# maybeLx/MVSFormerPlusPlus

Hardware: AMD Instinct MI355X
Metric: ref-views/sec at 1152x1536 N=5 D=192 4-stage; achieved HBM GB/s vs peak (higher is better)
Workload: dtype fp16 operands/storage, fp32 accumulate (every stage; 1-2 fp16 MFMA terms)

## Files before the change

mvsformerplusplus_amd/csrc/conv_bf16x3_kernels.hip:

```cpp
#include <map>
#include <mutex>
#include <type_traits>
#include <utility>

#include "conv_cfg.h"
#include "split_format.h"

#ifndef MVS_ABL
#define MVS_ABL 0
#endif
#ifndef MVS_WPF
#define MVS_WPF 1
#endif
#ifndef MVS_MSPLIT
#define MVS_MSPLIT 1
#endif
#ifndef MVS_MSPLIT_MIN_MREP
#define MVS_MSPLIT_MIN_MREP 4
#endif
#ifndef MVS_PERSIST
#define MVS_PERSIST 1
#endif
#ifndef MVS_PERSIST_PFD
#define MVS_PERSIST_PFD 1
// ... 613 lines not shown
}

#ifndef MVS_CONV_LOADER
#define MVS_CONV_LOADER 0
#endif
#if MVS_CONV_LOADER
__device__ float4 g_conv_zero_line[4];

template <class Cfg>
struct BfConvLd {
    static constexpr int OPT = BfConv<Cfg>::OPT;
    static constexpr int IMG = ((int)BfConv<Cfg>::LDS_BYTES + 255) / 256 * 256;
    static constexpr int NPC = (Cfg::NVOX + 63) / 64;
    static constexpr int NP = OPT * NPC;
    static constexpr size_t LDS_BYTES = (size_t)2 * IMG;
    static constexpr bool ENABLED = MVS_CONV_LOADER && BfConv<Cfg>::F16 && !BfConv<Cfg>::PERSIST && Cfg::KD == 3;
};

template <class Cfg>
__global__ __launch_bounds__(320) void conv3d_mfma_f16_loader_kernel(const _Float16* __restrict__ x, const void* wp, const float* __restrict__ bias,
                                                                     _Float16* __restrict__ y, int D, int H, int W, int OD, int OH, int OW,
                                                                     int relu, int tiles_x, int tiles_y, int ntiles) {
    constexpr int CIN = Cfg::CIN, COUT = Cfg::COUT, SD = Cfg::SD, SH = Cfg::SH, SW = Cfg::SW, TD = Cfg::TD, TH = Cfg::TH, CH = Cfg::CH;
    constexpr int IH = Cfg::IH, IW = Cfg::IW, MREP = Cfg::MREP, NREP = Cfg::NREP, NPASS = Cfg::NPASS, NVOX = Cfg::NVOX;
    constexpr int NSTEP = BfConv<Cfg>::NSTEP, SB = BfConv<Cfg>::SB, PLANE = BfConv<Cfg>::PLANE;
    constexpr int IMG = BfConvLd<Cfg>::IMG, NPC = BfConvLd<Cfg>::NPC, NP = BfConvLd<Cfg>::NP;
    static_assert(BfConv<Cfg>::F16 && SB == 16, "fp16 activations: 16 bytes per voxel and octet");
    HIP_DYNAMIC_SHARED(float4, lds4)
    char* lds = reinterpret_cast<char*>(lds4);
    const int tid = (int)threadIdx.x, lane = tid & 63;
    const int wave = __builtin_amdgcn_readfirstlane(tid >> 6);
    const int b = (int)blockIdx.y;
    const int nblk = (int)gridDim.x, per = (ntiles + nblk - 1) / nblk;
    const int t_begin = (int)xcd_remap(blockIdx.x, (unsigned)nblk) * per;
    const int t_end = t_begin + per < ntiles ? t_begin + per : ntiles;
    if (t_begin >= t_end) return;
    const int nchunk = (t_end - t_begin) * NPASS;
    const char* xb = reinterpret_cast<const char*>(x) + (size_t)b * D * H * W * CIN * 2;

    if (wave == 4) {
        const char* zero = reinterpret_cast<const char*>(g_conv_zero_line);
        int crd[NPC];
        int rel[NPC];
#pragma unroll
        for (int k = 0; k < NPC; ++k) {
            const int v = 64 * k + lane;
            const int dx = v % IW, t2 = v / IW, dy = t2 % IH, dz = t2 / IH;
            crd[k] = v < NVOX ? (dz << 16 | dy << 8 | dx) : -1;
            rel[k] = ((dz * H + dy) * W + dx) * (CIN * 2);
        }
        auto issue = [&](int c, int buf) {
            const int tile = t_begin + c / NPASS, pass = c - (c / NPASS) * NPASS;
            const int tx = tile % tiles_x, t1 = tile / tiles_x;
            const int ty = t1 % tiles_y, tz = t1 / tiles_y;
            const int iz0 = tz * TD * SD - Cfg::PD, iy0 = ty * TH * SH - 1, ix0 = tx * 16 * SW - 1;
            const long long base = ((long long)(iz0 * H + iy0) * W + ix0) * (CIN * 2) + pass * (CH * 2);
            char* img = lds + buf * IMG;
#pragma unroll
            for (int k = 0; k < NPC; ++k) {
                if (crd[k] < 0) continue;
                const int z = iz0 + (crd[k] >> 16), yy = iy0 + ((crd[k] >> 8) & 0xff), xx = ix0 + (crd[k] & 0xff);
                const bool ok = MVS_ABL != 1 && (unsigned)z < (unsigned)D && (unsigned)yy < (unsigned)H && (unsigned)xx < (unsigned)W;
#pragma unroll
                for (int oc = 0; oc < BfConvLd<Cfg>::OPT; ++oc) {
                    const char* src = ok ? xb + base + rel[k] + oc * 16 : zero;
                    MVS_GLOBAL_LOAD_LDS16(src, img + oc * PLANE + k * 1024);
                }
            }
        };
        issue(0, 0);
        MVS_WAIT_VMEM();
        __syncthreads();
        for (int c = 0; c < nchunk; ++c) {
            if (c + 1 < nchunk) issue(c + 1, (c + 1) & 1);
            MVS_WAIT_VMEM();
            __syncthreads();
        }
        return;
    }

    float sat_amax = 0.0f;
    const int li = lane & 15, g = lane >> 4;
    constexpr int MSPLIT = CfgSplit<Cfg>::MSPLIT, MREP_ALL = CfgSplit<Cfg>::MREP_ALL;
    const int mb0 = (wave % MSPLIT) * MREP, rowgrp = wave / MSPLIT;
    int voxbase[NREP];
#pragma unroll
    for (int nb = 0; nb < NREP; ++nb) {
        const int nbg = rowgrp * NREP + nb;
        const int oz = nbg / TH, oy = nbg % TH;
        voxbase[nb] = (((oz * SD) * IH + oy * SH) * IW + li * SW) * SB;
    }
    float4 bb[MREP];
#pragma unroll
    for (int mb = 0; mb < MREP; ++mb) {
        const int co = 16 * (mb0 + mb) + 4 * g;
        bb[mb] = co < COUT ? *reinterpret_cast<const float4*>(bias + co) : make_float4(0.0f, 0.0f, 0.0f, 0.0f);
    }
    _Float16* yb = y + (size_t)b * OD * OH * OW * COUT;
    f32x4 acc[MREP][NREP];
    __syncthreads();
    for (int c = 0; c < nchunk; ++c) {
        const int tile = t_begin + c / NPASS, pass = c - (c / NPASS) * NPASS;
        const char* cur = lds + (c & 1) * IMG;
        const bf16x8* wq = reinterpret_cast<const bf16x8*>(wp) + ((size_t)pass * NSTEP * MREP_ALL + mb0) * 2 * 64 + lane;
        bf16x8 ah[MVS_WPF + 1][MREP], al[MVS_WPF + 1][MREP];
        bf_conv_preload_w<Cfg>(wq, ah, al);
        if (pass == 0) {
#pragma unroll
            for (int mb = 0; mb < MREP; ++mb)
#pragma unroll
                for (int nb = 0; nb < NREP; ++nb) acc[mb][nb] = (f32x4){0.0f, 0.0f, 0.0f, 0.0f};
        }
        bf_conv_contract<Cfg>(wq, cur, voxbase, g, acc, ah, al);
        if (pass == NPASS - 1) {
            const int tx = tile % tiles_x, t1 = tile / tiles_x;
            const int ty = t1 % tiles_y, tz = t1 / tiles_y;
            const int oz0 = tz * TD, oy0 = ty * TH, ox0 = tx * 16;
#pragma unroll
            for (int nb = 0; nb < NREP; ++nb) {
                const int nbg = rowgrp * NREP + nb;
                const int oz = oz0 + nbg / TH, oy = oy0 + nbg % TH, ox = ox0 + li;
                if (!(oz < OD && oy < OH && ox < OW)) continue;
                _Float16* o = yb + (((size_t)oz * OH + oy) * OW + ox) * COUT;
#pragma unroll
                for (int mb = 0; mb < MREP; ++mb) {
                    const int co = 16 * (mb0 + mb) + 4 * g;
                    if (co >= COUT) continue;
                    float4 v = make_float4(acc[mb][nb][0] + bb[mb].x, acc[mb][nb][1] + bb[mb].y, acc[mb][nb][2] + bb[mb].z, acc[mb][nb][3] + bb[mb].w);
                    if (relu) { v.x = fmaxf(v.x, 0.0f); v.y = fmaxf(v.y, 0.0f); v.z = fmaxf(v.z, 0.0f); v.w = fmaxf(v.w, 0.0f); }
                    *reinterpret_cast<f16x4*>(o + co) = f16_pack4(v, sat_amax);
                }
            }
        }
        __syncthreads();
    }
    sat::commit(sat_amax);
}
#endif

template <class Cfg>
struct BfDeconv {
    static constexpr int OPT = Cfg::CIN / 8;
#ifndef MVS_DECONV_PLANES
#define MVS_DECONV_PLANES 1
#endif
    static constexpr bool F16 = CfgFmt<Cfg>::F16;
    static constexpr int RUNB = F16 ? 16 : 32;
    static constexpr int SB = F16 ? 16 : (MVS_DECONV_PLANES ? 32 : Cfg::S * 4);
    static constexpr int PLANE = F16 ? (Cfg::NVOX * 16 + 255) / 256 * 256 + bf_f16_plane_shift(1)
                                     : (MVS_DECONV_PLANES ? (Cfg::NVOX * 32 + 255) / 256 * 256 + 16 : 32);
    static constexpr size_t LDS_BYTES = (F16 || MVS_DECONV_PLANES) ? (size_t)OPT * PLANE : Cfg::LDS_BYTES;
};

template <class Cfg>
__device__ __forceinline__ void bf_deconv_load_step(int st, int ntap, int pd, int ph, int pw, int g, const bf16x8* wq, const char* ldsb,
                                                    const int* voxbase, bf16x8* ah, bf16x8* al, bf16x8* bh, bf16x8* bl) {
    constexpr int SD = Cfg::SD, OPT = BfDeconv<Cfg>::OPT;
    const int o = 4 * st + g;
    int ti = o / OPT;
    const int oc = o - ti * OPT;
    ti = ti < ntap ? ti : ntap - 1;
    const int nkw = pw ? 2 : 1, nkh = ph ? 2 : 1;
    const int a_w = ti % nkw;
    ti /= nkw;
    const int a_h = ti % nkh, a_d = ti / nkh;
    const int od = (SD == 2) ? (pd ? 1 - a_d : 0) : 1 - a_d;
    const int oh = ph ? 1 - a_h : 0, ow = pw ? 1 - a_w : 0;
    const int ldsoff = ((od * Cfg::LH + oh) * Cfg::LW + ow) * BfDeconv<Cfg>::SB + oc * BfDeconv<Cfg>::PLANE;
#pragma unroll
    for (int mb = 0; mb < Cfg::MREP; ++mb) {
        if (MVS_ABL == 2 && st > 1) continue;
        ah[mb] = wq[(size_t)((st * CfgSplit<Cfg>::MREP_ALL + mb) * 2) * 64];
        al[mb] = wq[(size_t)((st * CfgSplit<Cfg>::MREP_ALL + mb) * 2 + 1) * 64];
    }
#pragma unroll
    for (int nb = 0; nb < Cfg::NREP; ++nb) {
        if (MVS_ABL == 3 && st > 1) continue;
        bh[nb] = *reinterpret_cast<const bf16x8*>(ldsb + voxbase[nb] + ldsoff);
        if constexpr (!BfDeconv<Cfg>::F16) bl[nb] = *reinterpret_cast<const bf16x8*>(ldsb + voxbase[nb] + ldsoff + 16);
    }
}

template <class Cfg, bool SPLIT>
__global__ __launch_bounds__(256) void deconv3d_mfma_bf16x3_kernel(const float* __restrict__ x, const void* wp, const float* __restrict__ bias,
                                                                   const float* __restrict__ skip, float* __restrict__ y,
                                                                   const float* __restrict__ prob_w, const float* __restrict__ prob_b,
                                                                   float* __restrict__ logits, int D, int H, int W, int tiles_x,
                                                                   int tiles_y, int ntiles, int relu) {
    float sat_amax = 0.0f;
    constexpr int CIN = Cfg::CIN, COUT = Cfg::COUT, SD = Cfg::SD, TDM = Cfg::TDM, THM = Cfg::THM;
    constexpr int LH = Cfg::LH, LW = Cfg::LW, MREP = Cfg::MREP, NREP = Cfg::NREP;
    constexpr int OPT = BfDeconv<Cfg>::OPT, SB = BfDeconv<Cfg>::SB;
    const float lo_clamp = relu ? 0.0f : -INFINITY;
    HIP_DYNAMIC_SHARED(float4, lds4)
    char* ldsb = reinterpret_cast<char*>(lds4);
    const int tid = (int)threadIdx.x, lane = tid & 63, wave = tid >> 6;
    const int li = lane & 15, g = lane >> 4;
    start_stagger(2048);
    prio_kernel_begin();
    int tile = (int)xcd_remap(blockIdx.x, (unsigned)ntiles);
    const int b = (int)blockIdx.y;
    const int tx = tile % tiles_x;
    tile /= tiles_x;
    const int ty = tile % tiles_y, tz = tile / tiles_y;
    const int mz0 = tz * TDM, my0 = ty * THM, mx0 = tx * 16;
    const int OD = D * SD, OH = 2 * H, OW = 2 * W;

    constexpr bool F16 = BfDeconv<Cfg>::F16;
    constexpr int EB = F16 ? 2 : 4, RUNB = BfDeconv<Cfg>::RUNB;
    const char* xb = reinterpret_cast<const char*>(x) + (size_t)b * D * H * W * CIN * EB;
    {
        int zrel;
        const __amdgpu_buffer_rsrc_t xrs = bf_make_rsrc_z(xb, mz0 - Cfg::ZO, D, H, W, (unsigned)(CIN * EB), zrel);
        BfTileWalk<LW, LH, OPT, RUNB> wk(tid, zrel, my0, mx0, H, W, CIN * EB, 0u);
        int ldso = (tid / OPT) * SB + (tid % OPT) * BfDeconv<Cfg>::PLANE;
        for (int e = tid; e < Cfg::NVOX * OPT; e += 256) {
            const bool ok = MVS_ABL != 1 && wk.inside(mz0 - Cfg::ZO, my0, mx0, D, H, W);
            const unsigned voff = ok ? wk.off : BF_OOB;
            const float4 u = bf_buf_load16(xrs, voff, 0);
            if constexpr (F16) {
                *reinterpret_cast<float4*>(ldsb + ldso) = u;
            } else {
                const float4 v = bf_buf_load16(xrs, voff, 16);
                stage_to_lds<SPLIT>(ldsb + ldso, u, v);
            }
            wk.advance();
            ldso += (256 / OPT) * SB;
        }
    }
    __syncthreads();

    constexpr int MSPLIT = CfgSplit<Cfg>::MSPLIT, MREP_ALL = CfgSplit<Cfg>::MREP_ALL;
    const int mb0 = (wave % MSPLIT) * MREP, rowgrp = wave / MSPLIT;
    int voxbase[NREP];
#pragma unroll
    for (int nb = 0; nb < NREP; ++nb) {
        const int nbg = rowgrp * NREP + nb;
        const int mz = nbg / THM, my = nbg % THM;
        voxbase[nb] = (((mz + Cfg::ZO) * LH + my) * LW + li) * SB;
    }
    float* yb = reinterpret_cast<float*>(reinterpret_cast<char*>(y) + (size_t)b * OD * OH * OW * COUT * EB);
    const float* sb = skip ? reinterpret_cast<const float*>(reinterpret_cast<const char*>(skip) + (size_t)b * OD * OH * OW * COUT * EB) : nullptr;
    const bf16x8* wq = reinterpret_cast<const bf16x8*>(wp) + (size_t)mb0 * 2 * 64 + lane;

    constexpr bool PAIR = COUT == 8;
    constexpr int NCLS = (SD == 2 ? 2 : 1) * 4;
    constexpr int NIT = PAIR ? NCLS / 2 : NCLS;
    float4 skp[NIT][NREP][MREP];
    if (sb) {
#pragma unroll
        for (int it = 0; it < NIT; ++it) {
            const int cls = PAIR ? 2 * it : it;
            const int pw = PAIR ? 1 : (cls & 1), ph = (cls >> 1) & 1, pd = (SD == 2) ? (cls >> 2) : 0;
#pragma unroll
            for (int nb = 0; nb < NREP; ++nb) {
                const int nbg = rowgrp * NREP + nb;
                const int mz = mz0 + nbg / THM, my = my0 + nbg % THM, mx = mx0 + li;
                const bool inside = mz < D && my < H && mx < W;
                const int oz = mz * SD + pd, oy = 2 * my + ph, ox = PAIR ? 2 * mx + (g >> 1) : 2 * mx + pw;
#pragma unroll
                for (int mb = 0; mb < MREP; ++mb) {
                    const int co = PAIR ? 4 * (g & 1) : 16 * (mb0 + mb) + 4 * g;
                    const size_t sidx = (((size_t)oz * OH + oy) * OW + ox) * COUT;
                    const float* sv = sb + sidx;
                    if constexpr (F16) {
                        const float2 raw = !(inside && co < COUT) ? make_float2(0.0f, 0.0f)
                                                                  : *reinterpret_cast<const float2*>(reinterpret_cast<const _Float16*>(sb) + sidx + co);
                        skp[it][nb][mb] = make_float4(raw.x, raw.y, 0.0f, 0.0f);
                        continue;
                    }
                    skp[it][nb][mb] = !(inside && co < COUT) ? make_float4(0.0f, 0.0f, 0.0f, 0.0f)
                                      : SPLIT ? split_raw_quad(sv + (co & ~7), (co >> 2) & 1) : *reinterpret_cast<const float4*>(sv + co);
                }
            }
        }
    }
#pragma unroll
    for (int cls = 0; cls < NCLS; cls += PAIR ? 2 : 1) {
        const int it = PAIR ? cls / 2 : cls;
        const int pw = PAIR ? 1 : (cls & 1), ph = (cls >> 1) & 1, pd = (SD == 2) ? (cls >> 2) : 0;
        f32x4 acc[MREP][NREP];
#pragma unroll
        for (int mb = 0; mb < MREP; ++mb)
#pragma unroll
            for (int nb = 0; nb < NREP; ++nb) acc[mb][nb] = (f32x4){0.0f, 0.0f, 0.0f, 0.0f};
        const int ntap = ((SD == 2) ? (pd ? 2 : 1) : 3) * (ph ? 2 : 1) * (pw ? 2 : 1);
        const int nst = MVS_ABL == 6 ? 1 : (ntap * OPT + 3) / 4;
        bf16x8 ah0[MREP], al0[MREP], bh0[NREP], bl0[NREP], ah1[MREP], al1[MREP], bh1[NREP], bl1[NREP];
        prio_contract_begin();
        bf_deconv_load_step<Cfg>(0, ntap, pd, ph, pw, g, wq, ldsb, voxbase, ah0, al0, bh0, bl0);
#pragma unroll 1
        for (int st = 0; st + 1 < nst; st += 2) {
            bf_deconv_load_step<Cfg>(st + 1, ntap, pd, ph, pw, g, wq, ldsb, voxbase, ah1, al1, bh1, bl1);
            __builtin_amdgcn_sched_barrier(0);
            bf_mfma_step<MREP, NREP, F16>(ah0, al0, bh0, bl0, acc);
            bf_deconv_load_step<Cfg>(st + 2 < nst ? st + 2 : nst - 1, ntap, pd, ph, pw, g, wq, ldsb, voxbase, ah0, al0, bh0, bl0);
            __builtin_amdgcn_sched_barrier(0);
            bf_mfma_step<MREP, NREP, F16>(ah1, al1, bh1, bl1, acc);
        }
        if (nst & 1) bf_mfma_step<MREP, NREP, F16>(ah0, al0, bh0, bl0, acc);
        prio_contract_end();
        wq += (size_t)nst * MREP_ALL * 2 * 64;

#pragma unroll
        for (int nb = 0; nb < NREP; ++nb) {
            const int nbg = rowgrp * NREP + nb;
            const int mz = mz0 + nbg / THM, my = my0 + nbg % THM, mx = mx0 + li;
            const bool inside = mz < D && my < H && mx < W;
            if (!inside && !(PAIR && prob_w != nullptr) && !SPLIT) continue;
            if (PAIR) {
                const int oz = mz * SD + pd, oy = 2 * my + ph, ox = 2 * mx + (g >> 1), co = 4 * (g & 1);
                const size_t off = (((size_t)oz * OH + oy) * OW + ox) * COUT + co;
                const float4 bb = *reinterpret_cast<const float4*>(bias + co);
                float4 v = make_float4(fmaxf(acc[0][nb][0] + bb.x, lo_clamp), fmaxf(acc[0][nb][1] + bb.y, lo_clamp), fmaxf(acc[0][nb][2] + bb.z, lo_clamp),
                                       fmaxf(acc[0][nb][3] + bb.w, lo_clamp));
                if (sb && inside) {
                    const float4 sk = F16 ? f16_quad_to_f32(skp[it][nb][0]) : SPLIT ? split_join_quad(skp[it][nb][0]) : skp[it][nb][0];
                    v.x += sk.x; v.y += sk.y; v.z += sk.z; v.w += sk.w;
                }
                if (prob_w != nullptr) {
                    const float4 pw4 = *reinterpret_cast<const float4*>(prob_w + co);
                    float part = v.x * pw4.x;
                    part += v.y * pw4.y;
                    part += v.z * pw4.z;
                    part += v.w * pw4.w;
                    part += __shfl_xor(part, 16);
                    if ((g & 1) == 0 && inside && !(MVS_ABL == 5 && part != 12345.678f)) logits[(size_t)b * OD * OH * OW + ((size_t)oz * OH + oy) * OW + ox] = part + prob_b[0];
                } else if (F16) {
                    if (inside) *reinterpret_cast<f16x4*>(reinterpret_cast<_Float16*>(yb) + off) = f16_pack4(v, sat_amax);
                } else if (SPLIT) {
                    split_store_quad(yb + off - co, g, v, inside);
                } else {
                    if (!(MVS_ABL == 5 && v.x != 12345.678f)) *reinterpret_cast<float4*>(yb + off) = v;
                }
                continue;
            }
            const int oz = mz * SD + pd, oy = 2 * my + ph, ox = 2 * mx + pw;
            const size_t off = (((size_t)oz * OH + oy) * OW + ox) * COUT;
#pragma unroll
            for (int mb = 0; mb < MREP; ++mb) {
                const int co = 16 * (mb0 + mb) + 4 * g;
                if (!SPLIT && co >= COUT) continue;
                const float4 bb = *reinterpret_cast<const float4*>(bias + (co < COUT ? co : 0));
                float4 v = make_float4(fmaxf(acc[mb][nb][0] + bb.x, lo_clamp), fmaxf(acc[mb][nb][1] + bb.y, lo_clamp),
                                       fmaxf(acc[mb][nb][2] + bb.z, lo_clamp), fmaxf(acc[mb][nb][3] + bb.w, lo_clamp));
                if (sb) {
                    const float4 sk = F16 ? f16_quad_to_f32(skp[it][nb][mb]) : SPLIT ? split_join_quad(skp[it][nb][mb]) : skp[it][nb][mb];
                    v.x += sk.x; v.y += sk.y; v.z += sk.z; v.w += sk.w;
                }
                if (MVS_ABL == 5 && v.x != 12345.678f) continue;
                if constexpr (F16) *reinterpret_cast<f16x4*>(reinterpret_cast<_Float16*>(yb) + off + co) = f16_pack4(v, sat_amax);
                else if (SPLIT) split_store_quad(yb + off + (co & ~7), g, v, inside && co < COUT);
                else *reinterpret_cast<float4*>(yb + off + co) = v;
            }
        }
    }
    if constexpr (F16) sat::commit(sat_amax);
}

template <class Cfg>
struct BfDeconvP {
    static constexpr bool F16 = CfgFmt<Cfg>::F16;
    static constexpr int OPT = 2, SB = F16 ? 16 : 32, RUNB = SB;
    static constexpr int PLANE = F16 ? (Cfg::NVOX * 16 + 255) / 256 * 256 + bf_f16_plane_shift(1) : (Cfg::NVOX * 32 + 255) / 256 * 256 + 16;
    static constexpr int XBYTES = (2 * PLANE + 255) / 256 * 256;
    static constexpr int NIT = (Cfg::SD == 2 ? 2 : 1) * 2;
    static constexpr int ntap(int it) { return ((Cfg::SD == 2) ? ((it >> 1) ? 2 : 1) : 3) * ((it & 1) ? 2 : 1) * 2; }
    static constexpr int nst(int it) { return (ntap(it) * OPT + 3) / 4; }
    static constexpr int wbase(int it) { return it == 0 ? 0 : wbase(it - 1) + nst(it - 1); }
    static constexpr int WSTEPS = wbase(NIT);
    static constexpr int WBYTES = WSTEPS * 2048;
    static constexpr size_t LDS_BYTES = (size_t)XBYTES + WBYTES;
    static_assert(Cfg::CIN == 16 && Cfg::COUT == 8, "persistent deconv: the 16 -> 8 layer");
    static constexpr int tap_offset(int it, int o) {
        const int pd = (Cfg::SD == 2) ? (it >> 1) : 0, ph = it & 1;
        int ti = o / OPT;
        const int oc = o - ti * OPT;
        ti = ti < ntap(it) ? ti : ntap(it) - 1;
        const int a_w = ti % 2;
        ti /= 2;
        const int nkh = ph ? 2 : 1;
        const int a_h = ti % nkh, a_d = ti / nkh;
        const int od = (Cfg::SD == 2) ? (pd ? 1 - a_d : 0) : 1 - a_d;
        const int oh = ph ? 1 - a_h : 0, ow = 1 - a_w;
        return ((od * Cfg::LH + oh) * Cfg::LW + ow) * SB + oc * PLANE;
    }
};

template <class Cfg, int IT, int T>
__device__ __forceinline__ void bfd_load_step(int g, int lane, const char* ldsx, const char* ldsw, int voxbase0, bf16x8& ah, bf16x8& al, bf16x8* bh,
                                              bf16x8* bl) {
    using P = BfDeconvP<Cfg>;
    static_assert(Cfg::THM % Cfg::NREP == 0, "a wave's rows must stay inside one input plane");
    constexpr int ROWB = Cfg::LW * P::SB;
    constexpr int c0 = P::tap_offset(IT, 4 * T), c1 = P::tap_offset(IT, 4 * T + 1), c2 = P::tap_offset(IT, 4 * T + 2), c3 = P::tap_offset(IT, 4 * T + 3);
    int sel = c0;
    sel = g == 1 ? c1 : sel;
    sel = g == 2 ? c2 : sel;
    sel = g == 3 ? c3 : sel;
    const char* p = ldsx + voxbase0 + sel;
    const char* w = ldsw + (P::wbase(IT) + T) * 2048 + lane * 16;
    ah = *reinterpret_cast<const bf16x8*>(w);
    al = *reinterpret_cast<const bf16x8*>(w + 1024);
#pragma unroll
    for (int nb = 0; nb < Cfg::NREP; ++nb) {
        bh[nb] = *reinterpret_cast<const bf16x8*>(p + nb * ROWB);
        if constexpr (!P::F16) bl[nb] = *reinterpret_cast<const bf16x8*>(p + nb * ROWB + 16);
    }
}

template <class Cfg, int IT, int T>
struct BfDeconvSteps {
    static __device__ __forceinline__ void run(int g, int lane, const char* ldsx, const char* ldsw, int voxbase0, f32x4 (*acc)[Cfg::NREP], bf16x8* a0,
                                               bf16x8* bh0, bf16x8* bl0, bf16x8* a1, bf16x8* bh1, bf16x8* bl1) {
        constexpr int NST = BfDeconvP<Cfg>::nst(IT);
        if constexpr (T < NST) {
            if constexpr (T + 1 < NST) {
                if constexpr ((T & 1) == 0) bfd_load_step<Cfg, IT, T + 1>(g, lane, ldsx, ldsw, voxbase0, a1[0], a1[1], bh1, bl1);
                else bfd_load_step<Cfg, IT, T + 1>(g, lane, ldsx, ldsw, voxbase0, a0[0], a0[1], bh0, bl0);
            }
            __builtin_amdgcn_sched_barrier(0);
            if constexpr ((T & 1) == 0) bf_mfma_step<1, Cfg::NREP, CfgFmt<Cfg>::F16, CfgFmt<Cfg>::ONE>(&a0[0], &a0[1], bh0, bl0, acc);
            else bf_mfma_step<1, Cfg::NREP, CfgFmt<Cfg>::F16, CfgFmt<Cfg>::ONE>(&a1[0], &a1[1], bh1, bl1, acc);
            BfDeconvSteps<Cfg, IT, T + 1>::run(g, lane, ldsx, ldsw, voxbase0, acc, a0, bh0, bl0, a1, bh1, bl1);
        }
    }
};

template <class Cfg, bool SPLIT>
__global__ __launch_bounds__(256) void deconv3d_mfma_bf16x3_persist_kernel(const float* __restrict__ x, const void* wp, const float* __restrict__ bias,
                                                                           const float* __restrict__ skip, float* __restrict__ y,
                                                                           const float* __restrict__ prob_w, const float* __restrict__ prob_b,
                                                                           float* __restrict__ logits, int D, int H, int W, int tiles_x, int tiles_y,
                                                                           int ntiles, int relu) {
    float sat_amax = 0.0f;
    using P = BfDeconvP<Cfg>;
    const float lo_clamp = relu ? 0.0f : -INFINITY;
    constexpr int CIN = Cfg::CIN, COUT = Cfg::COUT, SD = Cfg::SD, TDM = Cfg::TDM, THM = Cfg::THM;
    constexpr int LH = Cfg::LH, LW = Cfg::LW, NREP = Cfg::NREP, NIT = P::NIT, OPT = P::OPT, SB = P::SB;
    HIP_DYNAMIC_SHARED(float4, lds4)
    char* ldsx = reinterpret_cast<char*>(lds4);
    char* ldsw = ldsx + P::XBYTES;
    const int tid = (int)threadIdx.x, lane = tid & 63, wave = tid >> 6;
    const int li = lane & 15, g = lane >> 4;
    const int b = (int)blockIdx.y;
    const int nblk = (int)gridDim.x, per = (ntiles + nblk - 1) / nblk;
    const int t_begin = (int)xcd_remap(blockIdx.x, (unsigned)nblk) * per;
    const int t_end = t_begin + per < ntiles ? t_begin + per : ntiles;
    if (t_begin >= t_end) return;
    const int OD = D * SD, OH = 2 * H, OW = 2 * W;

    for (int e = tid; e < P::WBYTES / 16; e += 256) reinterpret_cast<float4*>(ldsw)[e] = reinterpret_cast<const float4*>(wp)[e];

    constexpr bool F16 = P::F16;
    constexpr int EB = F16 ? 2 : 4;
// ... 65 lines not shown
#pragma unroll
        for (int it = 0; it < NITX; ++it) {
            const int e = tid + it * 256;
            if (e >= NITEM) break;
            const int vox = e / OPT, oc = e - vox * OPT;
            if constexpr (F16) *reinterpret_cast<float4*>(ldsx + vox * SB + oc * P::PLANE) = su[it];
            else stage_to_lds<SPLIT>(ldsx + vox * SB + oc * P::PLANE, su[it], sv[it]);
        }
        __syncthreads();
        if (tile + 1 < t_end) issue_x(tile + 1);

        const int tx = tile % tiles_x;
        const int t1 = tile / tiles_x;
        const int ty = t1 % tiles_y, tz = t1 / tiles_y;
        const int mz0 = tz * TDM, my0 = ty * THM, mx0 = tx * 16;
        float4 outv[NIT][NREP];
        auto run_class = [&](auto itc) {
            constexpr int IT = decltype(itc)::value;
            f32x4 acc[1][NREP];
#pragma unroll
            for (int nb = 0; nb < NREP; ++nb) acc[0][nb] = (f32x4){0.0f, 0.0f, 0.0f, 0.0f};
            bf16x8 a0[2], a1[2], bh0[NREP], bl0[NREP], bh1[NREP], bl1[NREP];
            bfd_load_step<Cfg, IT, 0>(g, lane, ldsx, ldsw, voxbase[0], a0[0], a0[1], bh0, bl0);
            BfDeconvSteps<Cfg, IT, 0>::run(g, lane, ldsx, ldsw, voxbase[0], acc, a0, bh0, bl0, a1, bh1, bl1);
#pragma unroll
            for (int nb = 0; nb < NREP; ++nb)
                outv[IT][nb] = make_float4(fmaxf(acc[0][nb][0] + bb.x, lo_clamp), fmaxf(acc[0][nb][1] + bb.y, lo_clamp), fmaxf(acc[0][nb][2] + bb.z, lo_clamp),
                                           fmaxf(acc[0][nb][3] + bb.w, lo_clamp));
        };
        run_class(std::integral_constant<int, 0>{});
        run_class(std::integral_constant<int, 1>{});
        if constexpr (NIT == 4) {
            run_class(std::integral_constant<int, 2>{});
            run_class(std::integral_constant<int, 3>{});
        }
#pragma unroll
        for (int it = 0; it < NIT; ++it) {
            const int pd = (SD == 2) ? (it >> 1) : 0, ph = it & 1;
#pragma unroll
            for (int nb = 0; nb < NREP; ++nb) {
                const int nbg = wave * NREP + nb;
                const int mz = mz0 + nbg / THM, my = my0 + nbg % THM, mx = mx0 + li;
                const bool inside = mz < D && my < H && mx < W;
                const int oz = mz * SD + pd, oy = 2 * my + ph, ox = 2 * mx + (g >> 1);
                float4 v = outv[it][nb];
                if (sb) {
                    const float4 sk = F16 ? f16_quad_to_f32(skp[it][nb]) : SPLIT ? split_join_quad(skp[it][nb]) : skp[it][nb];
                    v.x += sk.x; v.y += sk.y; v.z += sk.z; v.w += sk.w;
                }
                if (head) {
                    float part = v.x * pw4.x;
                    part += v.y * pw4.y;
                    part += v.z * pw4.z;
                    part += v.w * pw4.w;
                    part += __shfl_xor(part, 16);
                    if ((g & 1) == 0 && inside && !(MVS_ABL == 5 && part != 12345.678f))
                        logits[(size_t)b * OD * OH * OW + ((size_t)oz * OH + oy) * OW + ox] = part + pb;
                } else if (F16) {
                    if (inside) *reinterpret_cast<f16x4*>(reinterpret_cast<_Float16*>(yb) + (((size_t)oz * OH + oy) * OW + ox) * COUT + co) =
                        f16_pack4(v, sat_amax);
                } else if (SPLIT) {
                    split_store_quad(yb + (((size_t)oz * OH + oy) * OW + ox) * COUT, g, v, inside);
                } else if (inside && !(MVS_ABL == 5 && v.x != 12345.678f)) {
                    *reinterpret_cast<float4*>(yb + (((size_t)oz * OH + oy) * OW + ox) * COUT + co) = v;
                }
            }
        }
        if (sb && tile + 1 < t_end) issue_skip(tile + 1);
        __syncthreads();
    }
    if constexpr (F16) sat::commit(sat_amax);
}

static int resident_blocks(const void* func, size_t lds, int threads = 256) {
    static std::mutex mu;
    static std::map<std::pair<const void*, int>, int> cache;
    int dev = 0;
    if (hipGetDevice(&dev) != hipSuccess) return -1;
    std::lock_guard<std::mutex> lock(mu);
    auto it = cache.find(std::make_pair(func, dev));
    if (it != cache.end()) return it->second;
    int per_cu = 0;
    hipDeviceProp_t prop;
    if (lds > 48 * 1024) hipFuncSetAttribute(func, hipFuncAttributeMaxDynamicSharedMemorySize, (int)lds);
    if (hipGetDeviceProperties(&prop, dev) != hipSuccess || hipOccupancyMaxActiveBlocksPerMultiprocessor(&per_cu, func, threads, lds) != hipSuccess || per_cu < 1)
        return -1;
    return cache[std::make_pair(func, dev)] = per_cu * prop.multiProcessorCount;
}

template <class Cfg>
struct BfSplitOf {
    static constexpr bool SPLIT = MVS_MSPLIT && Cfg::MREP >= MVS_MSPLIT_MIN_MREP && Cfg::NREP <= 2 && Cfg::TH % (Cfg::NREP * 2) == 0;
    typedef typename std::conditional<SPLIT, SplitCfg<Cfg, 2>, Cfg>::type type;
};

template <class Cfg, bool SPLIT>
static int launch_conv_bf(const float* x, const void* wp, const float* bias, float* y, int B, int D, int H, int W, int relu, hipStream_t st,
                          float* logits) {
    const int OD = (D + 2 * Cfg::PD - Cfg::KD) / Cfg::SD + 1, OH = (H - 1) / Cfg::SH + 1, OW = (W - 1) / Cfg::SW + 1;
    const int tx = (int)ceil_div(OW, 16), ty = (int)ceil_div(OH, Cfg::TH), tz = (int)ceil_div(OD, Cfg::TD);
    const int ntiles = tx * ty * tz;
    constexpr size_t LDS = BfConv<Cfg>::PERSIST ? BfConv<Cfg>::PERSIST_LDS_BYTES : BfConv<Cfg>::LDS_BYTES;
    if constexpr (BfConv<Cfg>::PERSIST) {
        const int resident = resident_blocks(reinterpret_cast<const void*>(&conv3d_mfma_bf16x3_persist_kernel<Cfg, SPLIT>), LDS);
        if (resident < 1) { set_error("conv3d(bf16x3): occupancy query failed"); return MVS_ERR_LAUNCH; }
        const int nblk = ntiles < resident ? ntiles : resident;
        hipLaunchKernelGGL((conv3d_mfma_bf16x3_persist_kernel<Cfg, SPLIT>), dim3(nblk, B), dim3(256), LDS, st, x, wp, bias, y, logits, D, H, W, OD, OH, OW, relu, tx,
                           ty, ntiles);
        return check_launch("conv3d_mfma_bf16x3_persist_kernel");
    }
    if (logits != nullptr) { set_error("conv3d(bf16x3): the planar single-channel output needs a persistent (Cin = 8) kernel"); return MVS_ERR_UNSUPPORTED; }
#if MVS_CONV_LOADER
    if constexpr (BfConvLd<Cfg>::ENABLED) {
        static const bool off = getenv("MVS_CONV_LOADER_OFF") != nullptr;
        if (!off) {
            constexpr size_t LLDS = BfConvLd<Cfg>::LDS_BYTES;
            const int resident = resident_blocks(reinterpret_cast<const void*>(&conv3d_mfma_f16_loader_kernel<Cfg>), LLDS, 320);
            if (resident < 1) { set_error("conv3d(f16, loader): occupancy query failed"); return MVS_ERR_LAUNCH; }
            const int nblk = ntiles < resident ? ntiles : resident;
            hipLaunchKernelGGL((conv3d_mfma_f16_loader_kernel<Cfg>), dim3(nblk, B), dim3(320), LLDS, st, reinterpret_cast<const _Float16*>(x), wp, bias,
                               reinterpret_cast<_Float16*>(y), D, H, W, OD, OH, OW, relu, tx, ty, ntiles);
            return check_launch("conv3d_mfma_f16_loader_kernel");
        }
    }
#endif
    constexpr size_t TLDS = BfWlds<Cfg>::ENABLED ? BfWlds<Cfg>::LDS_BYTES : LDS;
    if (TLDS > 48 * 1024)
        hipFuncSetAttribute(reinterpret_cast<const void*>(&conv3d_mfma_bf16x3_kernel<Cfg, SPLIT>), hipFuncAttributeMaxDynamicSharedMemorySize, (int)TLDS);
    hipLaunchKernelGGL((conv3d_mfma_bf16x3_kernel<Cfg, SPLIT>), dim3(ntiles, B), dim3(256), TLDS, st, x, wp, bias, y, D, H, W, OD, OH, OW, relu, tx, ty, ntiles);
    return check_launch("conv3d_mfma_bf16x3_kernel");
}

template <class Cfg>
struct BfDeconvSplitOf {
    static constexpr bool SPLIT = MVS_MSPLIT && Cfg::MREP == 2 && Cfg::THM % (Cfg::NREP * 2) == 0;
    typedef typename std::conditional<SPLIT, SplitCfg<Cfg, 2>, Cfg>::type type;
};

template <class Cfg, bool SPLIT>
static int launch_deconv_bf(const float* x, const void* wp, const float* bias, const float* skip, float* y, const float* prob_w,
                            const float* prob_b, float* logits, int B, int D, int H, int W, hipStream_t st, int relu) {
    const int tx = (int)ceil_div(W, 16), ty = (int)ceil_div(H, Cfg::THM), tz = (int)ceil_div(D, Cfg::TDM);
    const int ntiles = tx * ty * tz;
    if constexpr (MVS_PERSIST && Cfg::CIN == 16 && Cfg::COUT == 8) {
        constexpr size_t LDS = BfDeconvP<Cfg>::LDS_BYTES;
        const int resident = resident_blocks(reinterpret_cast<const void*>(&deconv3d_mfma_bf16x3_persist_kernel<Cfg, SPLIT>), LDS);
        if (resident < 1) { set_error("deconv3d(bf16x3): occupancy query failed"); return MVS_ERR_LAUNCH; }
        const int nblk = ntiles < resident ? ntiles : resident;
        hipLaunchKernelGGL((deconv3d_mfma_bf16x3_persist_kernel<Cfg, SPLIT>), dim3(nblk, B), dim3(256), LDS, st, x, wp, bias, skip, y, prob_w, prob_b, logits, D, H,
                           W, tx, ty, ntiles, relu);
        return check_launch("deconv3d_mfma_bf16x3_persist_kernel");
    }
    constexpr size_t DLDS = BfDeconv<Cfg>::LDS_BYTES;
    if (DLDS > 48 * 1024)
        hipFuncSetAttribute(reinterpret_cast<const void*>(&deconv3d_mfma_bf16x3_kernel<Cfg, SPLIT>), hipFuncAttributeMaxDynamicSharedMemorySize, (int)DLDS);
    hipLaunchKernelGGL((deconv3d_mfma_bf16x3_kernel<Cfg, SPLIT>), dim3(ntiles, B), dim3(256), DLDS, st, x, wp, bias, skip, y, prob_w, prob_b,
                       logits, D, H, W, tx, ty, ntiles, relu);
    return check_launch("deconv3d_mfma_bf16x3_kernel");
}

static bool bf_input_fits(const char* who, int Cin, int D, int H, int W, int split) {
    const long long bytes = 12LL * H * W * Cin * (split >= 2 ? 2 : 4);
    if (bytes < (1LL << 31)) return true;
    set_error("%s: twelve z-planes of the input are %lld bytes; the MFMA convolutions address a tile's planes with 32-bit offsets (< 2 GB)", who, bytes);
    return false;
}

int conv3d_dispatch_bf16x3(const float* x, const void* wp, const float* bias, float* y, int B, int Cin, int Cout, int D, int H, int W,
                           int kd, int sd, int sh, int sw, int relu, hipStream_t st, float* logits, int split) {
    if (!bf_input_fits("conv3d(mfma)", Cin, D, H, W, split)) return MVS_ERR_UNSUPPORTED;
#define MVS_X(CI, CO, KD, SD, SH, SW, TD, TH, CH)                                                     \
    if (Cin == CI && Cout == CO && kd == KD && sd == SD && sh == SH && sw == SW) {                    \
        typedef typename BfSplitOf<ConvCfg<CI, CO, KD, SD, SH, SW, TD, TH, CH>>::type K;              \
        if (split == 3) return launch_conv_bf<F16x1Cfg<K>, false>(x, wp, bias, y, B, D, H, W, relu, st, logits); \
        if (split == 2) return launch_conv_bf<F16Cfg<K>, false>(x, wp, bias, y, B, D, H, W, relu, st, logits);   \
        return split ? launch_conv_bf<K, true>(x, wp, bias, y, B, D, H, W, relu, st, logits)          \
                     : launch_conv_bf<K, false>(x, wp, bias, y, B, D, H, W, relu, st, logits);        \
    }
    MVS_CONV_TABLE(MVS_X)
#undef MVS_X
    set_error("conv3d(bf16x3): no kernel for Cin=%d Cout=%d kernel=(%d,3,3) stride=(%d,%d,%d)", Cin, Cout, kd, sd, sh, sw);
    return MVS_ERR_UNSUPPORTED;
}

int deconv3d_dispatch_bf16x3(const float* x, const void* wp, const float* bias, const float* skip, float* y, int B, int Cin, int Cout,
                             int D, int H, int W, int sd, hipStream_t st, const float* prob_w, const float* prob_b, float* logits, int relu, int split) {
    if (prob_w != nullptr && Cout != 8) { set_error("deconv3d(bf16x3): the fused prob head needs Cout == 8"); return MVS_ERR_UNSUPPORTED; }
    if (!bf_input_fits("deconv3d(mfma)", Cin, D, H, W, split)) return MVS_ERR_UNSUPPORTED;
#define MVS_X(CI, CO, SD, TDM, THM)                                                                     \
    if (Cin == CI && Cout == CO && sd == SD) {                                                          \
        typedef typename BfDeconvSplitOf<DeconvCfg<CI, CO, SD, TDM, THM>>::type K;                      \
        if (split == 3) return launch_deconv_bf<F16x1Cfg<K>, false>(x, wp, bias, skip, y, prob_w, prob_b, logits, B, D, H, W, st, relu);    \
        if (split == 2) return launch_deconv_bf<F16Cfg<K>, false>(x, wp, bias, skip, y, prob_w, prob_b, logits, B, D, H, W, st, relu);      \
        return split ? launch_deconv_bf<K, true>(x, wp, bias, skip, y, prob_w, prob_b, logits, B, D, H, W, st, relu)    \
                     : launch_deconv_bf<K, false>(x, wp, bias, skip, y, prob_w, prob_b, logits, B, D, H, W, st, relu);  \
    }
    MVS_DECONV_TABLE(MVS_X)
#undef MVS_X
    set_error("deconv3d(bf16x3): no kernel for Cin=%d Cout=%d stride=(%d,2,2)", Cin, Cout, sd);
    return MVS_ERR_UNSUPPORTED;
}

}

namespace mvs { MVS_DEFINE_SAT_READER(sat_read_conv) }
```

Before: 677.9.

## Fuse deconv parity classes into one compile-time tap walk, drop low weight term

Adds a class-fused path for the stride-(1,2,2) transposed convolutions with 32 or 64 input channels. It walks the 27-tap neighbourhood once, loads each input fragment from LDS a single time, and feeds the MFMAs of all four output parity classes that use that tap, with weights fetched through buffer loads. Separately, when the format uses a single fp16 term, the low weight half is no longer loaded in the per-class path either. The aim is to cut repeated LDS reads and redundant weight loads. In exchange it needs four accumulator sets (more VGPRs, possibly lower occupancy) and a fully unrolled template walk that grows code size.

```diff
diff --git a/mvsformerplusplus_amd/csrc/conv_bf16x3_kernels.hip b/mvsformerplusplus_amd/csrc/conv_bf16x3_kernels.hip
--- a/mvsformerplusplus_amd/csrc/conv_bf16x3_kernels.hip
+++ b/mvsformerplusplus_amd/csrc/conv_bf16x3_kernels.hip
@@ -789,7 +789,7 @@
     static constexpr size_t LDS_BYTES = (F16 || MVS_DECONV_PLANES) ? (size_t)OPT * PLANE : Cfg::LDS_BYTES;
 };
 
-template <class Cfg>
+template <class Cfg, bool ONE = false>
 __device__ __forceinline__ void bf_deconv_load_step(int st, int ntap, int pd, int ph, int pw, int g, const bf16x8* wq, const char* ldsb,
                                                     const int* voxbase, bf16x8* ah, bf16x8* al, bf16x8* bh, bf16x8* bl) {
     constexpr int SD = Cfg::SD, OPT = BfDeconv<Cfg>::OPT;
@@ -808,7 +808,7 @@
     for (int mb = 0; mb < Cfg::MREP; ++mb) {
         if (MVS_ABL == 2 && st > 1) continue;
         ah[mb] = wq[(size_t)((st * CfgSplit<Cfg>::MREP_ALL + mb) * 2) * 64];
-        al[mb] = wq[(size_t)((st * CfgSplit<Cfg>::MREP_ALL + mb) * 2 + 1) * 64];
+        if constexpr (!ONE) al[mb] = wq[(size_t)((st * CfgSplit<Cfg>::MREP_ALL + mb) * 2 + 1) * 64];
     }
 #pragma unroll
     for (int nb = 0; nb < Cfg::NREP; ++nb) {
@@ -818,7 +818,128 @@
     }
 }
 
-template <class Cfg, bool SPLIT>
+#ifndef MVS_DECONV_ONE_TERM
+#define MVS_DECONV_ONE_TERM 1
+#endif
+#ifndef MVS_DECONV_FUSED_DEFAULT
+#define MVS_DECONV_FUSED_DEFAULT 1
+#endif
+#ifndef MVS_DECONV_WPF
+#define MVS_DECONV_WPF 0
+#endif
+template <class Cfg>
+struct BfDeconvF {
+    static constexpr bool ENABLED = Cfg::SD == 1 && (Cfg::CIN == 32 || Cfg::CIN == 64) && Cfg::COUT >= 16;
+    static constexpr bool F16 = CfgFmt<Cfg>::F16, ONE = MVS_DECONV_ONE_TERM && CfgFmt<Cfg>::ONE;
+    static constexpr bool DEFAULT = ENABLED && MVS_DECONV_FUSED_DEFAULT && ONE && Cfg::CIN == 64;
+    static constexpr int SPT = BfDeconv<Cfg>::OPT / 4;
+    static constexpr int NSTEP = 12 * SPT;
+    static constexpr int NW = MVS_DECONV_WPF + 1;
+    static constexpr int ROWB = Cfg::LW * BfDeconv<Cfg>::SB;
+    static constexpr bool uses(int cls, int p) { return ((cls & 2) || (p & 2)) && ((cls & 1) || (p & 1)); }
+    static constexpr int ntap(int cls) { return 3 * ((cls & 2) ? 2 : 1) * ((cls & 1) ? 2 : 1); }
+    static constexpr int wbase(int cls) { return cls == 0 ? 0 : wbase(cls - 1) + ntap(cls - 1) * SPT; }
+    static constexpr int wstep(int cls, int u) {
+        const int p = u / SPT, nkh = (cls & 2) ? 2 : 1, nkw = (cls & 1) ? 2 : 1;
+        const int a_d = p >> 2, a_h = (cls & 2) ? (p >> 1) & 1 : 0, a_w = (cls & 1) ? p & 1 : 0;
+        return wbase(cls) + ((a_d * nkh + a_h) * nkw + a_w) * SPT + u % SPT;
+    }
+    static constexpr int xoff(int u) {
+        const int p = u / SPT, od = 1 - (p >> 2), oh = 1 - ((p >> 1) & 1), ow = 1 - (p & 1);
+        return (((od + 1) * Cfg::LH + oh) * Cfg::LW + ow) * BfDeconv<Cfg>::SB + (u % SPT) * 4 * BfDeconv<Cfg>::PLANE;
+    }
+    static_assert(!ENABLED || Cfg::THM % Cfg::NREP == 0, "a wave's rows must stay inside one input plane");
+};
+
+template <class Cfg, int U, int CLS, int WHICH = 3, int WHEN = 0>
+__device__ __forceinline__ void bfdf_load_w(__amdgpu_buffer_rsrc_t wrs, unsigned wvoff, bf16x8* ah, bf16x8* al) {
+    using P = BfDeconvF<Cfg>;
+    constexpr bool prev = U > 0 && P::uses(CLS, (U > 0 ? U - 1 : 0) / P::SPT);
+    if constexpr (P::uses(CLS, U / P::SPT) && (WHEN == 0 || (WHEN == 1) == prev)) {
+        if (MVS_ABL == 2 && U > 1) return;
+#pragma unroll
+        for (int mb = 0; mb < Cfg::MREP; ++mb) {
+            constexpr int MREP_ALL = CfgSplit<Cfg>::MREP_ALL;
+            const int e = (P::wstep(CLS, U) * MREP_ALL + mb) * 2 * 1024;
+            if constexpr ((WHICH & 2) != 0) ah[mb] = __builtin_bit_cast(bf16x8, __builtin_amdgcn_raw_buffer_load_b128(wrs, (int)wvoff, e, 0));
+            if constexpr ((WHICH & 1) != 0 && !P::ONE) al[mb] = __builtin_bit_cast(bf16x8, __builtin_amdgcn_raw_buffer_load_b128(wrs, (int)wvoff, e + 1024, 0));
+        }
+    }
+}
+template <class Cfg, int U, int WHICH = 3, int WHEN = 0>
+__device__ __forceinline__ void bfdf_load_w_all(__amdgpu_buffer_rsrc_t wrs, unsigned wvoff, bf16x8 (*ah)[Cfg::MREP], bf16x8 (*al)[Cfg::MREP]) {
+    bfdf_load_w<Cfg, U, 0, WHICH, WHEN>(wrs, wvoff, ah[0], al[0]);
+    bfdf_load_w<Cfg, U, 1, WHICH, WHEN>(wrs, wvoff, ah[1], al[1]);
+    bfdf_load_w<Cfg, U, 2, WHICH, WHEN>(wrs, wvoff, ah[2], al[2]);
+    bfdf_load_w<Cfg, U, 3, WHICH, WHEN>(wrs, wvoff, ah[3], al[3]);
+}
+template <class Cfg, int U>
+__device__ __forceinline__ void bfdf_load_x(const char* px, bf16x8* bh, bf16x8* bl) {
+    using P = BfDeconvF<Cfg>;
+#pragma unroll
+    for (int nb = 0; nb < Cfg::NREP; ++nb) {
+        if (MVS_ABL == 3 && U > 1) continue;
+        bh[nb] = *reinterpret_cast<const bf16x8*>(px + P::xoff(U) + nb * P::ROWB);
+        if constexpr (!P::F16) bl[nb] = *reinterpret_cast<const bf16x8*>(px + P::xoff(U) + nb * P::ROWB + 16);
+    }
+}
+template <class Cfg, int U, int TERM, int CLS>
+__device__ __forceinline__ void bfdf_mfma(const bf16x8* ah, const bf16x8* al, const bf16x8* bh, const bf16x8* bl, f32x4 (*acc)[Cfg::NREP]) {
+    using P = BfDeconvF<Cfg>;
+    if constexpr (P::uses(CLS, U / P::SPT)) {
+#pragma unroll
+        for (int mb = 0; mb < Cfg::MREP; ++mb)
+#pragma unroll
+            for (int nb = 0; nb < Cfg::NREP; ++nb) {
+                if constexpr (P::F16)
+                    acc[mb][nb] = __builtin_amdgcn_mfma_f32_16x16x32_f16(__builtin_bit_cast(f16x8, TERM == 0 ? al[mb] : ah[mb]), __builtin_bit_cast(f16x8, bh[nb]),
+                                                                         acc[mb][nb], 0, 0, 0);
+                else
+                    acc[mb][nb] = __builtin_amdgcn_mfma_f32_16x16x32_bf16(TERM == 0 ? al[mb] : ah[mb], TERM == 1 ? bl[nb] : bh[nb], acc[mb][nb], 0, 0, 0);
+            }
+    }
+}
+template <class Cfg, int U, int TERM>
+__device__ __forceinline__ void bfdf_mfma_all(bf16x8 (*ah)[Cfg::MREP], bf16x8 (*al)[Cfg::MREP], const bf16x8* bh, const bf16x8* bl,
+                                              f32x4 (*acc)[Cfg::MREP][Cfg::NREP]) {
+    bfdf_mfma<Cfg, U, TERM, 0>(ah[0], al[0], bh, bl, acc[0]);
+    bfdf_mfma<Cfg, U, TERM, 1>(ah[1], al[1], bh, bl, acc[1]);
+    bfdf_mfma<Cfg, U, TERM, 2>(ah[2], al[2], bh, bl, acc[2]);
+    bfdf_mfma<Cfg, U, TERM, 3>(ah[3], al[3], bh, bl, acc[3]);
+}
+
+template <class Cfg, int U>
+struct BfDeconvFSteps {
+    using P = BfDeconvF<Cfg>;
+    static __device__ __forceinline__ void run(__amdgpu_buffer_rsrc_t wrs, unsigned wvoff, const char* px, f32x4 (*acc)[Cfg::MREP][Cfg::NREP],
+                                               bf16x8 (*ah)[4][Cfg::MREP], bf16x8 (*al)[4][Cfg::MREP], bf16x8 (*bh)[Cfg::NREP], bf16x8 (*bl)[Cfg::NREP]) {
+        constexpr int NSTEP = MVS_ABL == 6 ? 1 : P::NSTEP, WPF = MVS_DECONV_WPF, NW = P::NW;
+        constexpr bool NEXT = U + 1 < NSTEP;
+        if constexpr (U < NSTEP) {
+            if constexpr (WPF > 0 && U + WPF < NSTEP) bfdf_load_w_all<Cfg, U + WPF>(wrs, wvoff, ah[(U + WPF) % NW], al[(U + WPF) % NW]);
+            if constexpr (WPF == 0 && NEXT) bfdf_load_w_all<Cfg, U + 1, 3, 2>(wrs, wvoff, ah[0], al[0]);
+            if constexpr (NEXT) bfdf_load_x<Cfg, U + 1>(px, bh[(U + 1) & 1], bl[(U + 1) & 1]);
+            __builtin_amdgcn_sched_barrier(0);
+            if constexpr (!P::ONE) {
+                bfdf_mfma_all<Cfg, U, 0>(ah[U % NW], al[U % NW], bh[U & 1], bl[U & 1], acc);
+                if constexpr (WPF == 0 && NEXT) {
+                    __builtin_amdgcn_sched_barrier(0);
+                    bfdf_load_w_all<Cfg, U + 1, 1, 1>(wrs, wvoff, ah[0], al[0]);
+                    __builtin_amdgcn_sched_barrier(0);
+                }
+            }
+            if constexpr (!P::F16) bfdf_mfma_all<Cfg, U, 1>(ah[U % NW], al[U % NW], bh[U & 1], bl[U & 1], acc);
+            bfdf_mfma_all<Cfg, U, P::F16 ? 1 : 2>(ah[U % NW], al[U % NW], bh[U & 1], bl[U & 1], acc);
+            if constexpr (WPF == 0 && NEXT) {
+                __builtin_amdgcn_sched_barrier(0);
+                bfdf_load_w_all<Cfg, U + 1, 2, 1>(wrs, wvoff, ah[0], al[0]);
+            }
+            BfDeconvFSteps<Cfg, U + 1>::run(wrs, wvoff, px, acc, ah, al, bh, bl);
+        }
+    }
+};
+
+template <class Cfg, bool SPLIT, bool FUSED = false>
 __global__ __launch_bounds__(256) void deconv3d_mfma_bf16x3_kernel(const float* __restrict__ x, const void* wp, const float* __restrict__ bias,
                                                                    const float* __restrict__ skip, float* __restrict__ y,
                                                                    const float* __restrict__ prob_w, const float* __restrict__ prob_b,
@@ -912,32 +1033,62 @@
             }
         }
     }
+    constexpr bool ONE = MVS_DECONV_ONE_TERM && CfgFmt<Cfg>::ONE;
+    f32x4 accf[FUSED ? 4 : 1][MREP][NREP];
+    if constexpr (FUSED) {
+        using P = BfDeconvF<Cfg>;
+        static_assert(P::ENABLED && NCLS == 4 && !PAIR, "class-fused walk: the (1,2,2) layers with 32 / 64 input channels");
+#pragma unroll
+        for (int cls = 0; cls < 4; ++cls)
+#pragma unroll
+            for (int mb = 0; mb < MREP; ++mb)
+#pragma unroll
+                for (int nb = 0; nb < NREP; ++nb) accf[cls][mb][nb] = (f32x4){0.0f, 0.0f, 0.0f, 0.0f};
+        const __amdgpu_buffer_rsrc_t wrs = bf_make_rsrc(wp, (unsigned)(27 * P::SPT * MREP_ALL * 2 * 1024));
+        const unsigned wvoff = (unsigned)((mb0 * 2 * 64 + lane) * 16);
+        const char* px = ldsb + voxbase[0] - LH * LW * SB + g * BfDeconv<Cfg>::PLANE;
+        bf16x8 ah[P::NW][4][MREP], al[P::NW][4][MREP], bh[2][NREP], bl[2][NREP];
+        static_assert(MVS_DECONV_WPF >= 0 && MVS_DECONV_WPF <= 2, "weight prefetch distance of the class-fused walk");
+        prio_contract_begin();
+        bfdf_load_w_all<Cfg, 0>(wrs, wvoff, ah[0], al[0]);
+        if constexpr (MVS_DECONV_WPF > 1) bfdf_load_w_all<Cfg, 1>(wrs, wvoff, ah[1], al[1]);
+        bfdf_load_x<Cfg, 0>(px, bh[0], bl[0]);
+        BfDeconvFSteps<Cfg, 0>::run(wrs, wvoff, px, accf, ah, al, bh, bl);
+        prio_contract_end();
+    }
 #pragma unroll
     for (int cls = 0; cls < NCLS; cls += PAIR ? 2 : 1) {
         const int it = PAIR ? cls / 2 : cls;
         const int pw = PAIR ? 1 : (cls & 1), ph = (cls >> 1) & 1, pd = (SD == 2) ? (cls >> 2) : 0;
         f32x4 acc[MREP][NREP];
-#pragma unroll
-        for (int mb = 0; mb < MREP; ++mb)
-#pragma unroll
-            for (int nb = 0; nb < NREP; ++nb) acc[mb][nb] = (f32x4){0.0f, 0.0f, 0.0f, 0.0f};
-        const int ntap = ((SD == 2) ? (pd ? 2 : 1) : 3) * (ph ? 2 : 1) * (pw ? 2 : 1);
-        const int nst = MVS_ABL == 6 ? 1 : (ntap * OPT + 3) / 4;
-        bf16x8 ah0[MREP], al0[MREP], bh0[NREP], bl0[NREP], ah1[MREP], al1[MREP], bh1[NREP], bl1[NREP];
-        prio_contract_begin();
-        bf_deconv_load_step<Cfg>(0, ntap, pd, ph, pw, g, wq, ldsb, voxbase, ah0, al0, bh0, bl0);
+        if constexpr (FUSED) {
+#pragma unroll
+            for (int mb = 0; mb < MREP; ++mb)
+#pragma unroll
+                for (int nb = 0; nb < NREP; ++nb) acc[mb][nb] = accf[cls][mb][nb];
+        } else {
+#pragma unroll
+            for (int mb = 0; mb < MREP; ++mb)
+#pragma unroll
+                for (int nb = 0; nb < NREP; ++nb) acc[mb][nb] = (f32x4){0.0f, 0.0f, 0.0f, 0.0f};
+            const int ntap = ((SD == 2) ? (pd ? 2 : 1) : 3) * (ph ? 2 : 1) * (pw ? 2 : 1);
+            const int nst = MVS_ABL == 6 ? 1 : (ntap * OPT + 3) / 4;
+            bf16x8 ah0[MREP], al0[MREP], bh0[NREP], bl0[NREP], ah1[MREP], al1[MREP], bh1[NREP], bl1[NREP];
+            prio_contract_begin();
+            bf_deconv_load_step<Cfg, ONE>(0, ntap, pd, ph, pw, g, wq, ldsb, voxbase, ah0, al0, bh0, bl0);
 #pragma unroll 1
-        for (int st = 0; st + 1 < nst; st += 2) {
-            bf_deconv_load_step<Cfg>(st + 1, ntap, pd, ph, pw, g, wq, ldsb, voxbase, ah1, al1, bh1, bl1);
-            __builtin_amdgcn_sched_barrier(0);
-            bf_mfma_step<MREP, NREP, F16>(ah0, al0, bh0, bl0, acc);
-            bf_deconv_load_step<Cfg>(st + 2 < nst ? st + 2 : nst - 1, ntap, pd, ph, pw, g, wq, ldsb, voxbase, ah0, al0, bh0, bl0);
-            __builtin_amdgcn_sched_barrier(0);
-            bf_mfma_step<MREP, NREP, F16>(ah1, al1, bh1, bl1, acc);
-        }
-        if (nst & 1) bf_mfma_step<MREP, NREP, F16>(ah0, al0, bh0, bl0, acc);
-        prio_contract_end();
-        wq += (size_t)nst * MREP_ALL * 2 * 64;
+            for (int st = 0; st + 1 < nst; st += 2) {
+                bf_deconv_load_step<Cfg, ONE>(st + 1, ntap, pd, ph, pw, g, wq, ldsb, voxbase, ah1, al1, bh1, bl1);
+                __builtin_amdgcn_sched_barrier(0);
+                bf_mfma_step<MREP, NREP, F16, ONE>(ah0, al0, bh0, bl0, acc);
+                bf_deconv_load_step<Cfg, ONE>(st + 2 < nst ? st + 2 : nst - 1, ntap, pd, ph, pw, g, wq, ldsb, voxbase, ah0, al0, bh0, bl0);
+                __builtin_amdgcn_sched_barrier(0);
+                bf_mfma_step<MREP, NREP, F16, ONE>(ah1, al1, bh1, bl1, acc);
+            }
+            if (nst & 1) bf_mfma_step<MREP, NREP, F16, ONE>(ah0, al0, bh0, bl0, acc);
+            prio_contract_end();
+            wq += (size_t)nst * MREP_ALL * 2 * 64;
+        }
 
 #pragma unroll
         for (int nb = 0; nb < NREP; ++nb) {
@@ -1309,6 +1460,17 @@
         return check_launch("deconv3d_mfma_bf16x3_persist_kernel");
     }
     constexpr size_t DLDS = BfDeconv<Cfg>::LDS_BYTES;
+    if constexpr (BfDeconvF<Cfg>::ENABLED) {
+        const char* sw = getenv("MVS_DECONV_CLASS_FUSED");
+        const bool fused = (sw == nullptr || sw[0] == '\0') ? BfDeconvF<Cfg>::DEFAULT : sw[0] != '0';
+        if (fused) {
+            if (DLDS > 48 * 1024)
+                hipFuncSetAttribute(reinterpret_cast<const void*>(&deconv3d_mfma_bf16x3_kernel<Cfg, SPLIT, true>), hipFuncAttributeMaxDynamicSharedMemorySize, (int)DLDS);
+            hipLaunchKernelGGL((deconv3d_mfma_bf16x3_kernel<Cfg, SPLIT, true>), dim3(ntiles, B), dim3(256), DLDS, st, x, wp, bias, skip, y, prob_w, prob_b,
+                               logits, D, H, W, tx, ty, ntiles, relu);
+            return check_launch("deconv3d_mfma_bf16x3_kernel");
+        }
+    }
     if (DLDS > 48 * 1024)
         hipFuncSetAttribute(reinterpret_cast<const void*>(&deconv3d_mfma_bf16x3_kernel<Cfg, SPLIT>), hipFuncAttributeMaxDynamicSharedMemorySize, (int)DLDS);
     hipLaunchKernelGGL((deconv3d_mfma_bf16x3_kernel<Cfg, SPLIT>), dim3(ntiles, B), dim3(256), DLDS, st, x, wp, bias, skip, y, prob_w, prob_b,
```

Result: faster. 686.2, median of 6 (+1.2%).
